# darksim33/Pyneapple

Measured on AMD Instinct MI355X. Metric: voxels/sec (pixelwise triexp LM & 250-bin NNLS) at 1/2/4/8 MI355X, higher is better.
Workload: dtype f64

## Files before the change

pyneapple_amd/csrc/pnx_api.hip:

```cpp
#include <hip/hip_runtime.h>

#include <cmath>
#include <cstdarg>
#include <cstdio>
#include <cstring>
#include <algorithm>
#include <atomic>
#include <chrono>
#include <condition_variable>
#include <cstdlib>
#include <functional>
#include <mutex>
#include <string>
#include <thread>
#include <vector>

#include "pnx_curvefit_f32_kernel.hpp"
#include "pnx_curvefit_kernel.hpp"
#include "pnx_grid.hpp"
#include "pnx_grid_args.hpp"
#include "pnx_grid_posterior.hpp"
#include "pnx_grid_marginal.hpp"
#include "pnx_grid_prior.hpp"
#include "pnx_host_pipeline.hpp"
// ... 30 lines not shown
static constexpr int kQueueRing = 256;
static std::mutex g_mu;
static DeviceInfo g_dev[64];

static int get_device(int device, DeviceInfo **out) {
    int n = 0;
    if (hipGetDeviceCount(&n) != hipSuccess || n <= 0) return set_error(PNX_ERR_NO_DEVICE, "no HIP device visible");
    if (device < 0 || device >= n || device >= 64) return set_error(PNX_ERR_INVALID, "device %d out of range (%d visible)", device, n);
    std::lock_guard<std::mutex> lk(g_mu);
    DeviceInfo &d = g_dev[device];
    if (!d.ok) {
        hipDeviceProp_t prop;
        PNX_HIP(hipGetDeviceProperties(&prop, device));
        d.cus = prop.multiProcessorCount;
        PNX_HIP(hipSetDevice(device));
        PNX_HIP(hipMalloc(&d.queues, sizeof(unsigned long long) * kQueueRing));
        d.ok = true;
    }
    *out = &d;
    return PNX_OK;
}

static int use_device(int device, DeviceInfo **out) {
    if (int rc = get_device(device, out)) return rc;
    PNX_HIP(hipSetDevice(device));
    return PNX_OK;
}

static unsigned long long *next_queue(DeviceInfo *d) {
    std::lock_guard<std::mutex> lk(g_mu);
    unsigned long long *q = d->queues + d->next_queue;
    d->next_queue = (d->next_queue + 1) % kQueueRing;
    return q;
}

struct DevBuf {
    void *p = nullptr;
    ~DevBuf() {
        if (p) (void)hipFree(p);
    }
    int alloc(size_t bytes) {
        hipError_t e = hipMalloc(&p, bytes ? bytes : 8);
        if (e != hipSuccess) return set_error(PNX_ERR_NOMEM, "hipMalloc(%zu): %s", bytes, hipGetErrorString(e));
        return PNX_OK;
    }
};


struct HipBackend {
    typedef hipStream_t stream_t;
    typedef hipEvent_t event_t;
    static bool bind_device(int device) { return hipSetDevice(device) == hipSuccess; }
    static bool stream_create(stream_t *s, bool kernel) {
        int prio_least = 0, prio_greatest = 0;
        if (hipDeviceGetStreamPriorityRange(&prio_least, &prio_greatest) != hipSuccess) return false;
        const int prio_other = prio_least > 0 ? 0 : prio_greatest;
        return hipStreamCreateWithPriority(s, hipStreamNonBlocking, kernel ? prio_least : prio_other) == hipSuccess;
    }
    static void stream_destroy(stream_t s) { (void)hipStreamDestroy(s); }
    static bool stream_sync(stream_t s) { return hipStreamSynchronize(s) == hipSuccess; }
    static bool event_create(event_t *e) { return hipEventCreateWithFlags(e, hipEventDisableTiming) == hipSuccess; }
    static void event_destroy(event_t e) { (void)hipEventDestroy(e); }
    static bool event_record(event_t e, stream_t s) { return hipEventRecord(e, s) == hipSuccess; }
    static bool event_sync(event_t e) { return hipEventSynchronize(e) == hipSuccess; }
};
typedef PipeOpsT<hipStream_t> PipeOps;

static int run_pipeline(int n_chunks, int n_slots, int k_streams, int touchers, int device, hipStream_t user_stream,
                        const PipeOps &ops) {
    return run_pipeline_t<HipBackend>(n_chunks, n_slots, k_streams, touchers, device, user_stream, ops, dev_getenv("PNX_HOST_TRACE") != nullptr);
}

static void touch_pages(void *p, size_t bytes) {
    if (!p || !bytes) return;
    volatile char *c = (volatile char *)p;
    const uintptr_t a = (uintptr_t)p;
    c[0] = 0;
    for (size_t off = (4096 - (a & 4095)) & 4095; off < bytes; off += 4096) c[off] = 0;
}

int env_int(const char *name, int dflt, int lo, int hi) {
    const char *e = getenv(name);
    if (!e) return dflt;
    const long v = atol(e);
    return v < lo ? lo : (v > hi ? hi : (int)v);
}
const char *dev_getenv(const char *name) {
    static const bool enabled = [] {
        const char *e = getenv("PNX_ENABLE_TEST_HOOKS");
        return e && e[0] == '1' && e[1] == 0;
    }();
    return enabled ? getenv(name) : nullptr;
}
int dev_env_int(const char *name, int dflt, int lo, int hi) { return dev_getenv(name) ? env_int(name, dflt, lo, hi) : dflt; }

static std::atomic<int> g_host_calls(0);
struct HostCallGuard {
    int in_flight;
    HostCallGuard() : in_flight(g_host_calls.fetch_add(1) + 1) {}
    ~HostCallGuard() { g_host_calls.fetch_sub(1); }
    int touchers() const { return getenv("PNX_HOST_TOUCHERS") ? env_int("PNX_HOST_TOUCHERS", 2, 0, 8) : (in_flight >= 3 ? 0 : (in_flight == 2 ? 1 : 2)); }
    int out_threads() const { return getenv("PNX_STREAM_OUT_THREADS") ? env_int("PNX_STREAM_OUT_THREADS", 2, 1, 4) : (in_flight >= 4 ? 1 : 2); }
};

struct Carver {
    char *base = nullptr;
    size_t off = 0;
    void *take(size_t bytes) {
        void *p = base ? base + off : nullptr;
        off += (bytes + 255) & ~(size_t)255;
        return p;
    }
};

static int model_n_params(int model) {
    switch (model) {
    case PNX_MODEL_MONO: return 2;
    case PNX_MODEL_BI_REDUCED: return 3;
    case PNX_MODEL_BI_S0: return 4;
    case PNX_MODEL_BI_FULL: return 4;
    case PNX_MODEL_TRI_REDUCED: return 5;
    case PNX_MODEL_TRI_S0: return 6;
    case PNX_MODEL_TRI_FULL: return 6;
    }
    return -1;
}

typedef int (*launch_fn)(int, int, const CurvefitArgs *, int, void *);
static launch_fn g_launch[7] = {pnx_launch_curvefit_m0, pnx_launch_curvefit_m1, pnx_launch_curvefit_m2,
                                pnx_launch_curvefit_m3, pnx_launch_curvefit_m4, pnx_launch_curvefit_m5,
                                pnx_launch_curvefit_m6};

struct StreamLaunch {
    StreamCtl *ctl = nullptr;
    unsigned int *host_flags = nullptr;
    int granule_shift = 0;
    unsigned int spins = 0;
    int phase = 0;
};

static int curvefit_device(const pnx_curvefit_opts *o, int64_t n_vox, const double *b, const double *y_d,
                           const double *p0, const double *lo, const double *hi, const double *fixed, double *popt_d,
                           double *pcov_d, int8_t *status_d, int32_t *nfev_d, double *cost_d, DeviceInfo *dev,
                           hipStream_t stream, const StreamLaunch *sl = nullptr, const int32_t *order = nullptr) {
    CurvefitArgs a;
    memset(&a, 0, sizeof(a));
    if (sl) {
        a.ctl = sl->ctl;
        a.host_flags = sl->host_flags;
        a.granule_shift = sl->granule_shift;
        a.stream_spins = sl->spins;
        a.phase = sl->phase;
    }
    a.order = sl ? nullptr : order;
    a.y = y_d;
    a.popt = popt_d;
    a.pcov = pcov_d;
    a.status = status_d;
    a.nfev = nfev_d;
    a.cost = cost_d;
    a.n_vox = n_vox;
    a.n_b = o->n_b;
    a.per_voxel = o->per_voxel_p0_bounds;
    a.fixed_per_voxel = o->fixed_per_voxel;
    a.max_nfev = o->max_nfev > 0 ? o->max_nfev : 100 * o->n_free;
    a.n_fixed = o->n_fixed;
    a.t1_mode = o->t1_mode;
    a.tr = o->tr;
    a.tm = o->tm;
    a.ftol = o->ftol;
    a.xtol = o->xtol;
    a.gtol = o->gtol;
    for (int k = 0; k < o->n_free; ++k) a.free_idx[k] = o->free_idx[k];
    for (int k = 0; k < o->n_fixed; ++k) a.fixed_idx[k] = o->fixed_idx[k];
    for (int i = 0; i < o->n_b; ++i) a.b[i] = b[i];
    a.absolute_sigma = o->absolute_sigma != 0;
    a.use_sigma = o->sigma != nullptr;
    if (o->sigma)
        for (int i = 0; i < o->n_b; ++i) a.w[i] = 1.0 / o->sigma[i];
    if (o->per_voxel_p0_bounds) {
        a.p0 = p0;
        a.lo = lo;
        a.hi = hi;
    } else {
        for (int k = 0; k < o->n_free; ++k) {
            a.p0s[k] = p0[k];
            a.los[k] = lo[k];
            a.his[k] = hi[k];
        }
    }
    if (o->n_fixed) {
        if (o->fixed_per_voxel)
            a.fixed = fixed;
        else
            for (int k = 0; k < o->n_fixed; ++k) a.fixeds[k] = fixed[k];
    }
    if (a.phase != 2) {
        a.queue = next_queue(dev);
        PNX_HIP(hipMemsetAsync(a.queue, 0, sizeof(unsigned long long), stream));
    }
    return g_launch[o->model](o->n_free, o->jac_mode, &a, dev->cus, (void *)stream);
}

static int check_curvefit_opts(const pnx_curvefit_opts *o) {
    if (!o) return set_error(PNX_ERR_INVALID, "opts is NULL");
    int n_all = model_n_params(o->model);
    if (n_all < 0) return set_error(PNX_ERR_INVALID, "unknown model %d", o->model);
    if (o->t1_mode < 0 || o->t1_mode > 2) return set_error(PNX_ERR_INVALID, "t1_mode %d", o->t1_mode);
    if (o->t1_mode) n_all += 1;
    if (o->n_b < 1 || o->n_b > PNX_MAX_BVALUES) return set_error(PNX_ERR_INVALID, "n_b=%d out of range [1,%d]", o->n_b, PNX_MAX_BVALUES);
    if (o->n_free < 1 || o->n_fixed < 0 || o->n_free + o->n_fixed != n_all)
        return set_error(PNX_ERR_INVALID, "n_free=%d + n_fixed=%d != %d parameters of model %d", o->n_free, o->n_fixed, n_all, o->model);
    bool seen[PNX_MAX_PARAMS] = {false};
    for (int k = 0; k < o->n_free; ++k) {
        const int j = o->free_idx[k];
        if (j < 0 || j >= n_all || seen[j] || (k && j <= o->free_idx[k - 1]))
            return set_error(PNX_ERR_INVALID, "free_idx must be ascending, unique positions in [0,%d)", n_all);
        seen[j] = true;
    }
    for (int k = 0; k < o->n_fixed; ++k) {
        const int j = o->fixed_idx[k];
        if (j < 0 || j >= n_all || seen[j]) return set_error(PNX_ERR_INVALID, "fixed_idx overlaps free_idx or is out of range");
        seen[j] = true;
    }
    if (o->jac_mode != PNX_JAC_FD && o->jac_mode != PNX_JAC_ANALYTIC) return set_error(PNX_ERR_INVALID, "jac_mode %d", o->jac_mode);
    if (o->jac_mode == PNX_JAC_FD && o->n_fixed)
        return set_error(PNX_ERR_UNSUPPORTED,
                         "finite-difference Jacobian with fixed parameters: the reference uses the analytic Jacobian "
                         "there (curvefit.py:274-288); pass PNX_JAC_ANALYTIC");
    if (!(o->ftol >= 0) || !(o->xtol >= 0) || !(o->gtol >= 0)) return set_error(PNX_ERR_INVALID, "tolerances must be >= 0");
    return PNX_OK;
}

}

using namespace pnx;

extern "C" {

int pnx_version(void) { return PNX_VERSION_MAJOR * 100 + PNX_VERSION_MINOR; }

int pnx_device_count(void) {
    int n = 0;
    if (hipGetDeviceCount(&n) != hipSuccess) return 0;
    return n;
}

int pnx_last_error(char *buf, int n) {
    const int len = (int)strlen(g_err);
    if (buf && n > 0) {
        strncpy(buf, g_err, (size_t)n - 1);
        buf[n - 1] = 0;
    }
    return len;
}

int pnx_model_n_params(int model) {
    const int n = model_n_params(model);
    return n < 0 ? set_error(PNX_ERR_INVALID, "unknown model %d", model) : n;
}

}

template <typename S, typename D> __global__ void cvt_kernel(const S *__restrict__ src, D *__restrict__ dst, size_t n) {
    for (size_t i = (size_t)blockIdx.x * blockDim.x + threadIdx.x; i < n; i += (size_t)gridDim.x * blockDim.x)
        dst[i] = (D)src[i];
}
template <typename S, typename D> static int cvt(const S *src, D *dst, size_t n, hipStream_t st) {
    if (!n) return PNX_OK;
    size_t blocks = (n + 255) / 256;
    if (blocks > 16384) blocks = 16384;
    hipLaunchKernelGGL((cvt_kernel<S, D>), dim3((unsigned)blocks), dim3(256), 0, st, src, dst, n);
    PNX_HIP(hipGetLastError());
    return PNX_OK;
}

struct AsyncBuf {
    void *p = nullptr;
    hipStream_t st = nullptr;
    int alloc(size_t bytes, hipStream_t s) {
        st = s;
        hipError_t e = hipMallocAsync(&p, bytes ? bytes : 8, s);
        if (e != hipSuccess) return set_error(PNX_ERR_NOMEM, "hipMallocAsync(%zu): %s", bytes, hipGetErrorString(e));
        return PNX_OK;
    }
    ~AsyncBuf() {
        if (p) (void)hipFreeAsync(p, st);
    }
};

struct DevSet {
    void *dev[ArrayTable::kMax] = {};
    void *xfer[ArrayTable::kMax] = {};
    double *d(int k) const { return (double *)dev[k]; }
};
enum class Carve { Staged, Results, CallerDevice };
static void carve(Carver &cv, const ArrayTable &A, size_t cap, DevSet &D, Carve mode = Carve::Staged, size_t v0 = 0) {
    for (int k = 0; k < A.n; ++k) {
        const HostArray &a = A.a[k];
        D.dev[k] = D.xfer[k] = nullptr;
        if (mode == Carve::CallerDevice) {
            if (!a.host) continue;
            D.xfer[k] = (char *)a.host + v0 * a.w * a.esize;
            D.dev[k] = a.widen ? cv.take(cap * a.w * sizeof(double)) : D.xfer[k];
        } else if ((a.host || a.always) && (a.out || mode == Carve::Staged)) {
            D.dev[k] = cv.take(cap * a.w * (a.widen ? sizeof(double) : a.esize));
// ... 1606 lines not shown
```

pyneapple_amd/csrc/pnx_curvefit_kernel.hpp:

```cpp
#pragma once
#include <hip/hip_runtime.h>
#include <stdint.h>

#include "pnx_trf_math.hpp"

namespace pnx {

constexpr int kWave = 64;
constexpr int kMaxB = 128;
constexpr int kMaxP = 8;
#ifdef PNX_ROW_BLK
template <int N> constexpr int row_blk() { return PNX_ROW_BLK; }
#else
template <int N> constexpr int row_blk() { return N >= 7 ? 2 : (N >= 5 ? 4 : 8); }
#endif
constexpr double kEps = TrfTraits<double>::eps;
constexpr double kSqrtEps = 1.4901161193847656e-08;
template <bool B> struct BoolC {
    static constexpr bool value = B;
};
typedef __attribute__((address_space(3))) void lds_void;

struct StreamCtl {
    unsigned long long ready;
    unsigned int abort;
    unsigned int timed_out;
    unsigned int done[1];
};

struct CurvefitArgs {
    const double *y;
    const double *p0;
    const double *lo;
    const double *hi;
    const double *fixed;
    double *popt;
    double *pcov;
    int8_t *status;
    int32_t *nfev;
    double *cost;
    unsigned long long *queue;
    const int32_t *order;
    StreamCtl *ctl;
    unsigned int *host_flags;
    int granule_shift;
    unsigned int stream_spins;
    int phase;
    long long n_vox;
    int n_b;
    int per_voxel;
    int fixed_per_voxel;
    int max_nfev;
    int n_fixed;
    int t1_mode;
    double tr, tm;
    double ftol, xtol, gtol;
    double p0s[kMaxP], los[kMaxP], his[kMaxP], fixeds[kMaxP];
    int free_idx[kMaxP];
    int fixed_idx[kMaxP];
    int use_sigma;
    int absolute_sigma;
    double b[kMaxB];
    double w[kMaxB];
};

template <int MODEL> struct Model;

template <> struct Model<0> {
    static constexpr int NALL = 2, NC = 1;
    __device__ static constexpr int dpos(int c) { return 1; }
    __device__ static double signal(const double *p, const double *E) { return p[0] * E[0]; }
    __device__ static void jac(const double *p, const double *E, double x, double *r) {
        r[0] = E[0];
        r[1] = -x * p[0] * E[0];
    }
};
template <> struct Model<1> {
    static constexpr int NALL = 3, NC = 2;
    __device__ static constexpr int dpos(int c) { return c == 0 ? 1 : 2; }
    __device__ static double signal(const double *p, const double *E) { return p[0] * E[0] + (1 - p[0]) * E[1]; }
    __device__ static void jac(const double *p, const double *E, double x, double *r) {
        r[0] = E[0] - E[1];
        r[1] = -x * p[0] * E[0];
        r[2] = -x * (1 - p[0]) * E[1];
    }
};
template <> struct Model<2> {
    static constexpr int NALL = 4, NC = 2;
    __device__ static constexpr int dpos(int c) { return c == 0 ? 1 : 2; }
    __device__ static double signal(const double *p, const double *E) {
        return p[3] * (p[0] * E[0] + (1 - p[0]) * E[1]);
    }
    __device__ static void jac(const double *p, const double *E, double x, double *r) {
        r[0] = p[3] * (E[0] - E[1]);
        r[1] = -x * p[3] * p[0] * E[0];
        r[2] = -x * p[3] * (1 - p[0]) * E[1];
        r[3] = p[0] * E[0] + (1 - p[0]) * E[1];
    }
};
template <> struct Model<3> {
    static constexpr int NALL = 4, NC = 2;
    __device__ static constexpr int dpos(int c) { return c == 0 ? 1 : 3; }
    __device__ static double signal(const double *p, const double *E) { return p[0] * E[0] + p[2] * E[1]; }
    __device__ static void jac(const double *p, const double *E, double x, double *r) {
        r[0] = E[0];
        r[1] = -x * p[0] * E[0];
        r[2] = E[1];
        r[3] = -x * p[2] * E[1];
    }
};
template <> struct Model<4> {
    static constexpr int NALL = 5, NC = 3;
    __device__ static constexpr int dpos(int c) { return c == 0 ? 1 : (c == 1 ? 3 : 4); }
    __device__ static double signal(const double *p, const double *E) {
        return p[0] * E[0] + p[2] * E[1] + (1 - p[0] - p[2]) * E[2];
    }
    __device__ static void jac(const double *p, const double *E, double x, double *r) {
        const double f3 = 1 - p[0] - p[2];
        r[0] = E[0] - E[2];
        r[1] = -x * p[0] * E[0];
        r[2] = E[1] - E[2];
        r[3] = -x * p[2] * E[1];
        r[4] = -x * f3 * E[2];
    }
};
template <> struct Model<5> {
    static constexpr int NALL = 6, NC = 3;
    __device__ static constexpr int dpos(int c) { return c == 0 ? 1 : (c == 1 ? 3 : 4); }
    __device__ static double signal(const double *p, const double *E) {
        return p[5] * (p[0] * E[0] + p[2] * E[1] + (1 - p[0] - p[2]) * E[2]);
    }
    __device__ static void jac(const double *p, const double *E, double x, double *r) {
        const double f3 = 1 - p[0] - p[2], S0 = p[5];
        r[0] = S0 * (E[0] - E[2]);
        r[1] = -x * S0 * p[0] * E[0];
        r[2] = S0 * (E[1] - E[2]);
        r[3] = -x * S0 * p[2] * E[1];
        r[4] = -x * S0 * f3 * E[2];
        r[5] = p[0] * E[0] + p[2] * E[1] + f3 * E[2];
    }
};
template <> struct Model<6> {
    static constexpr int NALL = 6, NC = 3;
    __device__ static constexpr int dpos(int c) { return c == 0 ? 1 : (c == 1 ? 3 : 5); }
    __device__ static double signal(const double *p, const double *E) {
        return p[0] * E[0] + p[2] * E[1] + p[4] * E[2];
    }
    __device__ static void jac(const double *p, const double *E, double x, double *r) {
        r[0] = E[0];
        r[1] = -x * p[0] * E[0];
        r[2] = E[1];
        r[3] = -x * p[2] * E[1];
        r[4] = E[2];
        r[5] = -x * p[4] * E[2];
    }
};

template <int MODEL> __host__ __device__ constexpr int colperm(int k) {
    constexpr int P[7][6] = {{0, 1, 2, 3, 4, 5}, {2, 0, 1, 3, 4, 5}, {2, 0, 1, 3, 4, 5}, {3, 1, 2, 0, 4, 5},
                             {4, 3, 0, 2, 1, 5}, {4, 3, 0, 2, 1, 5}, {5, 3, 1, 4, 2, 0}};
    return P[MODEL][k];
}

template <int MODEL> __device__ constexpr int comp_of_param(int j) {
    for (int c = 0; c < Model<MODEL>::NC; ++c)
        if (Model<MODEL>::dpos(c) == j) return c;
    return -1;
}

#ifndef PNX_CF_FAST_EXP
#define PNX_CF_FAST_EXP 1
#endif
#ifndef PNX_CF_HINTS
#define PNX_CF_HINTS 1
#endif
#if PNX_CF_HINTS
#define PNX_LIKELY(x) __builtin_expect(!!(x), 1)
#else
#define PNX_LIKELY(x) (x)
#endif
__device__ inline double exp_fast(double x) {
#if PNX_CF_FAST_EXP
    const double k = __builtin_rint(x * 1.4426950408889634);
    double r = fma(k, -0.6931471805599453, x);
    r = fma(k, -2.3190468138462996e-17, r);
    const double r2 = r * r;
    double qe = 2.7630903490112654e-07;
    qe = fma(qe, r2, 2.480149103909504e-05);
    qe = fma(qe, r2, 0.0013888888945916382);
    qe = fma(qe, r2, 0.041666666666519754);
    qe = fma(qe, r2, 0.5000000000000012);
    double qo = 2.502232256764614e-08;
    qo = fma(qo, r2, 2.755751454582531e-06);
    qo = fma(qo, r2, 0.00019841269589115522);
    qo = fma(qo, r2, 0.008333333333455043);
    qo = fma(qo, r2, 0.16666666666666477);
    const double q = fma(r, qo, qe);
    return ldexp(fma(r, fma(r, q, 1.0), 1.0), __double2int_rz(k));
#else
    return exp(x);
#endif
}

enum LaneState : int { ST_IDLE = 0, ST_INIT = 1, ST_RUN = 2, ST_FINAL = 3 };

template <int N> struct Park {
    static constexpr int NR = N * (N + 1) / 2;
    static constexpr bool kParkV = (N <= 5);
    static constexpr int NV = kParkV ? N * N : 0;
    __host__ __device__ static constexpr int per_wave(int tile_rows) { return kWave * (tile_rows + NR + NV); }
    __host__ __device__ static constexpr int per_wave_f64(int n_b) { return kWave * (((n_b + 1) & ~1) + NR + NV); }
};

#ifndef PNX_CF_WAVES_PER_SIMD
#define PNX_CF_WAVES_PER_SIMD 1
#endif
#ifndef PNX_CF_BLOCK_WAVES
#define PNX_CF_BLOCK_WAVES 4
#endif
template <int MODEL, int N, bool FD, bool PV, bool T1, bool STREAM = false>
__global__ void __launch_bounds__(64 * PNX_CF_BLOCK_WAVES, PNX_CF_WAVES_PER_SIMD) curvefit_kernel(const CurvefitArgs A) {
    using M = Model<MODEL>;
    using PK = Park<N>;
    constexpr int NALL = M::NALL;
    constexpr int NP = NALL + (T1 ? 1 : 0);
    constexpr int NC = M::NC;
    constexpr bool HASFIXED = (N != NP);
    static_assert(!(FD && HASFIXED), "finite-difference mode is only built without fixed parameters");
    auto CP = [](int k) constexpr { return (HASFIXED || k >= NALL) ? k : colperm<MODEL>(k); };

    extern __shared__ double smem[];
    const int n_b = A.n_b;
    double *bsh = smem;
    const int lane = threadIdx.x & (kWave - 1);
    const int wave = threadIdx.x / kWave;
    const bool use_w = A.use_sigma != 0;
    const double *wsh = smem + kMaxB;
    double *ytile = smem + (use_w ? 2 * kMaxB : kMaxB) + (size_t)wave * PK::per_wave_f64(n_b);
    double *ysh = ytile + 2 * lane;
    double *rpark = ytile + (size_t)((n_b + 1) & ~1) * kWave + lane;
    double *vpark = rpark + (size_t)PK::NR * kWave;
    for (int i = threadIdx.x; i < n_b; i += blockDim.x) bsh[i] = A.b[i];
    if (use_w)
        for (int i = threadIdx.x; i < n_b; i += blockDim.x) smem[kMaxB + i] = A.w[i];
    double bmax = 0;
    for (int i = 0; i < n_b; ++i) {
        const double ab = fabs(A.b[i]);
        bmax = (ab < INFINITY) ? fmax(bmax, ab) : INFINITY;
    }
    __syncthreads();
    const bool dma_ok = ((reinterpret_cast<uintptr_t>(A.y) & 7) == 0);

    int state = ST_IDLE;
    long long vox = -1;
    unsigned long long ready_seen = 0;
    int pub = 0;
    auto publish = [&](bool all) {
        const int n_gran = (int)((A.n_vox + (1ll << A.granule_shift) - 1) >> A.granule_shift);
        int upto = pub;
        while (upto < n_gran && (all || !__ballot(state != ST_IDLE && (vox >> A.granule_shift) <= upto))) ++upto;
        if (upto == pub) return;
        __builtin_amdgcn_fence(__ATOMIC_RELEASE, "");
        const unsigned int n_waves = gridDim.x * (blockDim.x / kWave);
        if ((threadIdx.x & (kWave - 1)) == __ffsll((unsigned long long)__ballot(1)) - 1) {
            for (int g = pub; g < upto; ++g) {
                const unsigned int old = __hip_atomic_fetch_add(&A.ctl->done[g], 1u, __ATOMIC_ACQ_REL, __HIP_MEMORY_SCOPE_SYSTEM);
                if (old + 1 == n_waves) __hip_atomic_store(&A.host_flags[g], 1u, __ATOMIC_RELEASE, __HIP_MEMORY_SCOPE_SYSTEM);
            }
        }
        pub = upto;
    };
    double x[N], lb[N], ub[N];
    double pfull[NP];
    double g[N];
    double s[N], uf[N], R2[N][N], d[N], g_h[N];
    double Vreg[PK::kParkV ? 1 : N][PK::kParkV ? 1 : N];
    double smax = 0, smin = 0, theta = 0;
    double cost = 0, Delta = 0, alpha = 0;
    int nfev = 0, term = -99;
    bool first = false;
    double xn[N], step_h_norm = 0, step_norm = 0, predicted = 0;
    if (!PV) {
#pragma unroll
        for (int k = 0; k < N; ++k) {
            lb[k] = A.los[k];
            ub[k] = A.his[k];
        }
    }

#ifdef PNX_CF_STAMP
    unsigned long long seg[8] = {0, 0, 0, 0, 0, 0, 0, 0}, act[8] = {0, 0, 0, 0, 0, 0, 0, 0}, cnt[8] = {0, 0, 0, 0, 0, 0, 0, 0};
    unsigned long long tl = __builtin_amdgcn_s_memtime();
#define CFSTAMP(k) do { __builtin_amdgcn_s_waitcnt(0); const unsigned long long t_ = __builtin_amdgcn_s_memtime(); seg[k] += t_ - tl; tl = t_; } while (0)
#define CFACT(k, cond) do { act[k] += __popcll(__ballot(cond)); cnt[k] += 1; } while (0)
#else
#define CFSTAMP(k) do {} while (0)
#define CFACT(k, cond) do {} while (0)
#endif
    auto refill = [&]() {
    while (state == ST_IDLE) {
        const unsigned long long idx = atomicAdd(A.queue, 1ULL);
        if (idx >= (unsigned long long)A.n_vox) break;
        if constexpr (STREAM) {
            if (idx >= ready_seen) {
                bool got = false;
                const unsigned int *abort_word = A.host_flags + ((A.n_vox + (1ll << A.granule_shift) - 1) >> A.granule_shift);
                for (unsigned int spins = 0; spins < A.stream_spins; ++spins) {
                    ready_seen = __hip_atomic_load(&A.ctl->ready, __ATOMIC_ACQUIRE, __HIP_MEMORY_SCOPE_SYSTEM);
                    if (idx < ready_seen) {
                        got = true;
                        break;
                    }
                    if ((spins & 15u) == 15u && __hip_atomic_load(abort_word, __ATOMIC_RELAXED, __HIP_MEMORY_SCOPE_SYSTEM)) break;
                    __builtin_amdgcn_s_sleep(127);
                }
                if (!got) {
                    if (!__hip_atomic_load(abort_word, __ATOMIC_RELAXED, __HIP_MEMORY_SCOPE_SYSTEM))
                        __hip_atomic_store(&A.ctl->timed_out, 1u, __ATOMIC_RELAXED, __HIP_MEMORY_SCOPE_SYSTEM);
                    break;
                }
            }
        }
        vox = (long long)idx;
        if constexpr (!STREAM) {
            if (A.order) vox = A.order[idx];
        }
        const double *yv = A.y + (size_t)vox * n_b;
        if (dma_ok) {
            const int pairs = n_b >> 1;
            for (int c = 0; c < pairs; ++c)
                __builtin_amdgcn_global_load_lds((const void *)(yv + 2 * c), (lds_void *)(ytile + c * 2 * kWave), 16, 0, 0);
            if (n_b & 1) {
                if (vox + 1 < A.n_vox)
                    __builtin_amdgcn_global_load_lds((const void *)(yv + n_b - 1), (lds_void *)(ytile + pairs * 2 * kWave), 16, 0, 0);
                else
                    ysh[pairs * 2 * kWave] = yv[n_b - 1];
            }
        } else {
            for (int i = 0; i < n_b; ++i) ysh[(i >> 1) * 2 * kWave + (i & 1)] = yv[i];
        }
        bool okb = true, okp = true;
        double p0v[N];
#pragma unroll
        for (int k = 0; k < N; ++k) {
            if (PV) {
                p0v[k] = A.p0[(size_t)k * A.n_vox + vox];
                lb[k] = A.lo[(size_t)k * A.n_vox + vox];
                ub[k] = A.hi[(size_t)k * A.n_vox + vox];
            } else
                p0v[k] = A.p0s[k];
            okb = okb && (lb[k] < ub[k]);
            okp = okp && (p0v[k] >= lb[k]) && (p0v[k] <= ub[k]);
        }
        if (HASFIXED) {
#pragma unroll
            for (int j = 0; j < NP; ++j) pfull[j] = 0;
            for (int f = 0; f < A.n_fixed; ++f) {
                const double fv = A.fixed_per_voxel ? A.fixed[(size_t)f * A.n_vox + vox] : A.fixeds[f];
#pragma unroll
                for (int j = 0; j < NP; ++j)
                    if (A.fixed_idx[f] == j) pfull[j] = fv;
            }
        }
        if (!okb || !okp) {
            const int st = !okb ? -1 : -3;
#pragma unroll
            for (int k = 0; k < N; ++k) A.popt[(size_t)k * A.n_vox + vox] = p0v[k];
            if (A.status) A.status[vox] = (int8_t)st;
            if (A.nfev) A.nfev[vox] = 0;
            if (A.cost) A.cost[vox] = NAN;
            continue;
        }
#pragma unroll
        for (int k = 0; k < N; ++k) xn[k] = strictly_feasible_r(p0v[k], lb[k], ub[k]);
        state = ST_INIT;
        nfev = 0;
        term = -99;
        alpha = 0.0;
    }
    };
    refill();
    if constexpr (STREAM) {
        if (!__ballot(state != ST_IDLE)) publish(true);
    }
    for (;;) {
        CFSTAMP(7);
        if (state == ST_IDLE) break;
        asm volatile("s_waitcnt vmcnt(0)" ::: "memory");
        CFSTAMP(0);
        CFACT(1, true);

        double Rn[N][N], qn[N], gn[N], cost_new = 0;
        bool finite_f = true, yfinite = true;
        {
            double pe[NP];
            if (HASFIXED) {
#pragma unroll
                for (int j = 0; j < NP; ++j) {
                    pe[j] = pfull[j];
#pragma unroll
                    for (int k = 0; k < N; ++k)
                        if (A.free_idx[k] == j) pe[j] = xn[k];
                }
            } else {
#pragma unroll
                for (int j = 0; j < NP; ++j) pe[j] = xn[j];
            }
            double dxv[N];
            if (FD) {
#pragma unroll
                for (int k = 0; k < N; ++k) {
                    const double sign = (xn[k] >= 0) ? 1.0 : -1.0;
                    double h = kSqrtEps * sign * fmax(1.0, fabs(xn[k]));
                    const double lower_dist = xn[k] - lb[k], upper_dist = ub[k] - xn[k];
                    const double xx = xn[k] + h;
                    const bool violated = (xx < lb[k]) || (xx > ub[k]);
                    const bool fitting = fabs(h) <= fmax(lower_dist, upper_dist);
                    if (violated && fitting) h = -h;
                    if (!fitting) h = (upper_dist >= lower_dist) ? upper_dist : -lower_dist;
                    dxv[k] = (xn[k] + h) - xn[k];
                }
            }
            double A1 = 1.0, eTM = 1.0, fac = 1.0, dfac = 0.0;
            if (T1) {
                const bool steam = A.t1_mode == 2;
                const double T1v = pe[NALL];
                const double eTR = exp(-A.tr / T1v);
                A1 = 1 - eTR;
                eTM = steam ? exp(-A.tm / T1v) : 1.0;
                fac = A1 * eTM;
                dfac = steam ? eTM / (T1v * T1v) * (-A.tr * eTR + A.tm * A1) : (-eTR * A.tr / (T1v * T1v));
                if (FD) {
                    const double dx = dxv[N - 1];
                    const double T2 = T1v + dx;
                    const double fac2 = (1 - exp(-A.tr / T2)) * (steam ? exp(-A.tm / T2) : 1.0);
                    dfac = (fac2 - fac) / dx;
                }
            }
#pragma unroll
            for (int i = 0; i < N; ++i) {
                qn[i] = 0;
                gn[i] = 0;
#pragma unroll
                for (int j = 0; j < N; ++j) Rn[i][j] = 0;
            }
            constexpr int kRowBlk = row_blk<N>();
            static_assert(kRowBlk % 2 == 0, "a block reads its signal values as [pair][lane][2] pairs");
            auto row_block = [&](auto fastgz_c, auto usew_c, auto tail_c, const int i0) __attribute__((always_inline)) {
                constexpr bool FASTGZ = decltype(fastgz_c)::value, USEW = decltype(usew_c)::value, TAIL = decltype(tail_c)::value;
                double blk[kRowBlk][N + 1];
                double bv[TAIL ? 1 : kRowBlk], yv[TAIL ? 1 : kRowBlk];
                if constexpr (!TAIL) {
#pragma unroll
                    for (int r = 0; r < kRowBlk; r += 2) {
                        const double2 b2 = *reinterpret_cast<const double2 *>(bsh + i0 + r);
                        const double2 y2 = *reinterpret_cast<const double2 *>(ysh + (size_t)(i0 + r) * kWave);
                        bv[r] = b2.x;
                        bv[r + 1] = b2.y;
                        yv[r] = y2.x;
                        yv[r + 1] = y2.y;
                    }
                }
#pragma unroll
                for (int r = 0; r < kRowBlk; ++r) {
                    const bool live = !TAIL || (i0 + r < n_b);
                    const int ii = live ? i0 + r : 0;
                    const double bb = TAIL ? bsh[ii] : bv[TAIL ? 0 : r];
                    const double nb = -bb;
                    const double yi = TAIL ? ysh[(ii >> 1) * 2 * kWave + (ii & 1)] : yv[TAIL ? 0 : r];
                    yfinite = yfinite && isfinite(yi);
                    double E[NC];
#pragma unroll
                    for (int c = 0; c < NC; ++c) E[c] = exp_fast(nb * pe[M::dpos(c)]);
                    const double base = M::signal(pe, E);
                    double r0 = (T1 ? base * A1 * eTM : base) - yi;
                    double jr[N];
                    {
                        double ja[NP];
                        M::jac(pe, E, bb, ja);
                        if (FD) {
#pragma unroll
                            for (int k = 0; k < NALL; ++k) {
                                if (comp_of_param<MODEL>(k) >= 0) {
                                    const double z = nb * dxv[k];
                                    double gz;
#if PNX_CF_FAST_EXP
                                    if (FASTGZ || PNX_LIKELY(fabs(z) < 2e-4))
                                        gz = fma(z, fma(z, fma(z, 1.0 / 24, 1.0 / 6), 0.5), 1.0);
                                    else
#endif
                                    if (fabs(z) < 1e-3)
                                        gz = 1.0 + z * (0.5 + z * (1.0 / 6 + z * (1.0 / 24 + z * (1.0 / 120 + z * (1.0 / 720)))));
                                    else
                                        gz = expm1(z) / z;
                                    ja[k] *= gz;
                                }
                            }
                        }
                        if (T1) {
#pragma unroll
                            for (int k = 0; k < NALL; ++k) ja[k] *= fac;
                            ja[NP - 1] = base * dfac;
                        }
                        if (TAIL ? use_w : USEW) {
                            const double t = wsh[ii];
                            r0 *= t;
#pragma unroll
                            for (int k = 0; k < NP; ++k) ja[k] *= t;
                        }
                        if (HASFIXED) {
#pragma unroll
                            for (int k = 0; k < N; ++k) {
                                jr[k] = 0;
#pragma unroll
                                for (int j = 0; j < NP; ++j)
                                    if (A.free_idx[k] == j) jr[k] = ja[j];
                            }
                        } else {
#pragma unroll
                            for (int k = 0; k < N; ++k) jr[k] = ja[k];
                        }
                    }
                    const double rr = live ? r0 : 0.0;
                    finite_f = finite_f && isfinite(rr);
                    cost_new += rr * rr;
#pragma unroll
                    for (int k = 0; k < N; ++k) {
                        const double jk = live ? jr[k] : 0.0;
                        gn[k] += jk * rr;
                    }
#pragma unroll
                    for (int k = 0; k < N; ++k) blk[r][k] = live ? jr[CP(k)] : 0.0;
                    blk[r][N] = rr;
                }
                CFSTAMP(1);
                qr_merge<N, kRowBlk>(Rn, qn, blk);
                CFSTAMP(6);
            };
            auto row_loop = [&](auto fastgz_c, auto usew_c) __attribute__((always_inline)) {
                int i0 = 0;
                for (; i0 + kRowBlk <= n_b; i0 += kRowBlk) row_block(fastgz_c, usew_c, BoolC<false>{}, i0);
                if (i0 < n_b) row_block(BoolC<false>{}, BoolC<false>{}, BoolC<true>{}, i0);
            };
            constexpr bool kOneLoop = (N >= 6);
            bool gz_cubic = FD && PNX_CF_FAST_EXP && !kOneLoop;
            if (FD && PNX_CF_FAST_EXP && !kOneLoop) {
                bool in_range = true;
#pragma unroll
                for (int k = 0; k < NALL; ++k)
                    if (comp_of_param<MODEL>(k) >= 0) in_range = in_range && (fabs(bmax * dxv[k]) < 2e-4);
                gz_cubic = __ballot(!in_range) == 0;
            }
            if constexpr (kOneLoop) {
                for (int i0 = 0; i0 < n_b; i0 += kRowBlk) row_block(BoolC<false>{}, BoolC<false>{}, BoolC<true>{}, i0);
            } else if (PNX_LIKELY(!use_w && (gz_cubic || !FD))) {
                if constexpr (FD && PNX_CF_FAST_EXP)
                    row_loop(BoolC<true>{}, BoolC<false>{});
                else
                    row_loop(BoolC<false>{}, BoolC<false>{});
            } else if (use_w) {
                row_loop(BoolC<false>{}, BoolC<true>{});
            } else {
                if constexpr (FD) row_loop(BoolC<false>{}, BoolC<false>{});
            }
            cost_new *= 0.5;
        }

        CFSTAMP(1);
        bool accepted = false;
        int final_status = 0;
        if (state == ST_INIT) {
            if (!finite_f) {
                final_status = yfinite ? -4 : -2;
                cost = NAN;
                nfev = 0;
                state = ST_FINAL;
            } else {
                accepted = true;
                nfev = 1;
                first = true;
                state = ST_RUN;
            }
        } else {
            nfev += 1;
            if (!finite_f) {
                Delta = 0.25 * step_h_norm;
            } else {
                const double actual = cost - cost_new;
                double ratio;
                if (predicted > 0)
                    ratio = actual / predicted;
                else if (predicted == 0 && actual == 0)
                    ratio = 1;
                else
                    ratio = 0;
                double Delta_new = Delta;
                if (ratio < 0.25)
                    Delta_new = 0.25 * step_h_norm;
                else if (ratio > 0.75 && step_h_norm > 0.95 * Delta)
                    Delta_new = Delta * 2.0;
                const bool ftol_ok = (actual < A.ftol * cost) && (ratio > 0.25);
                const bool xtol_ok = step_norm < A.xtol * (A.xtol + normn<N>(x));
                if (ftol_ok && xtol_ok)
                    term = 4;
                else if (ftol_ok)
                    term = 2;
                else if (xtol_ok)
                    term = 3;
                if (term == -99) {
                    alpha *= Delta / Delta_new;
                    Delta = Delta_new;
                }
                accepted = actual > 0;
            }
        }
        if (accepted) {
#pragma unroll
            for (int i = 0; i < N; ++i) {
                x[i] = xn[i];
                g[i] = gn[i];
            }
            cost = cost_new;
            int t = 0;
#pragma unroll
            for (int i = 0; i < N; ++i)
#pragma unroll
                for (int j = i; j < N; ++j) rpark[(t++) * kWave] = Rn[i][j];
        }

        double v[N], dv[N], g_norm = 0;
        if (state == ST_RUN && (accepted || term != -99 || nfev >= A.max_nfev)) {
#pragma unroll
            for (int i = 0; i < N; ++i) {
                v[i] = 1.0;
                dv[i] = 0.0;
                if (g[i] < 0 && isfinite(ub[i])) {
                    v[i] = ub[i] - x[i];
                    dv[i] = -1;
                }
                if (g[i] > 0 && isfinite(lb[i])) {
                    v[i] = x[i] - lb[i];
                    dv[i] = 1;
                }
                g_norm = fmax(g_norm, fabs(g[i] * v[i]));
            }
            if (first) {
                double t = 0;
#pragma unroll
                for (int i = 0; i < N; ++i) {
                    const double q = x[i] / sqrt(v[i]);
                    t += q * q;
                }
                Delta = sqrt(t);
                if (Delta == 0) Delta = 1.0;
                first = false;
            }
            if (g_norm < A.gtol) term = 1;
            if (term != -99 || nfev >= A.max_nfev) {
                final_status = (term == -99) ? 0 : term;
                state = ST_FINAL;
            }
        }

        CFSTAMP(2);
        CFACT(3, state == ST_FINAL);
        if (state == ST_FINAL) {
            const bool ok = final_status > 0;
#pragma unroll
            for (int k = 0; k < N; ++k) {
                const double pk = ok ? x[k] : (PV ? A.p0[(size_t)k * A.n_vox + vox] : A.p0s[k]);
                A.popt[(size_t)k * A.n_vox + vox] = pk;
            }
            if (A.status) A.status[vox] = (int8_t)final_status;
            if (A.nfev) A.nfev[vox] = nfev;
            if (A.cost) A.cost[vox] = cost;
            if (A.pcov && ok) {
                double *pc = A.pcov + (size_t)vox * N * N;
#pragma unroll
                for (int t = 0; t < PK::NR; ++t) pc[t] = rpark[t * kWave];
            }
            state = ST_IDLE;
        }
        CFACT(0, state == ST_IDLE);
        if constexpr (STREAM) {
            const bool any_idle = __ballot(state == ST_IDLE) != 0;
            if (state == ST_IDLE) refill();
            if (any_idle) publish(false);
        } else {
            if (state == ST_IDLE) refill();
        }

        CFSTAMP(3);
        CFACT(4, state == ST_RUN && accepted);
        CFACT(5, state == ST_RUN);
        if (state == ST_RUN) {
            if (accepted) {
                double diag_h[N];
#pragma unroll
                for (int i = 0; i < N; ++i) {
                    d[i] = sqrt(v[i]);
                    diag_h[i] = g[i] * dv[i];
                    g_h[i] = d[i] * g[i];
                }
                double q2[N];
                double blk[N][N + 1];
#pragma unroll
                for (int i = 0; i < N; ++i) {
                    q2[i] = qn[i];
#pragma unroll
                    for (int j = 0; j < N; ++j) {
                        R2[i][j] = (j >= i) ? Rn[i][j] * d[CP(j)] : 0.0;
                        blk[i][j] = (i == j) ? sqrt(diag_h[CP(i)]) : 0.0;
                    }
                    blk[i][N] = 0.0;
                }
                qr_merge<N, N>(R2, q2, blk);
                double W[N][N], Vw[N][N];
#pragma unroll
                for (int i = 0; i < N; ++i)
#pragma unroll
                    for (int j = 0; j < N; ++j) W[i][j] = (i >= j) ? R2[j][i] : 0.0;
                jacobi_svd<N>(W, Vw);
                smax = 0;
                smin = INFINITY;
#pragma unroll
                for (int k = 0; k < N; ++k) {
                    double nn = 0, dq = 0;
#pragma unroll
                    for (int i = 0; i < N; ++i) {
                        nn += W[i][k] * W[i][k];
                        dq += Vw[i][k] * q2[i];
                    }
                    double inv = 0.0;
                    if (nn > 0) nn = fast_sqrt_rsqrt(nn, &inv);
                    s[k] = nn;
                    uf[k] = dq;
#pragma unroll
                    for (int i = 0; i < N; ++i) {
                        if (PK::kParkV)
                            vpark[(i * N + k) * kWave] = W[i][k] * inv;
                        else
                            Vreg[PK::kParkV ? 0 : i][PK::kParkV ? 0 : k] = W[i][k] * inv;
                    }
                    smax = fmax(smax, nn);
                    smin = fmin(smin, nn);
                }
                theta = fmax(0.995, 1 - g_norm);
            }
            CFSTAMP(4);
            double V[N][N];
#pragma unroll
            for (int i = 0; i < N; ++i)
#pragma unroll
                for (int k = 0; k < N; ++k)
                    V[i][k] = PK::kParkV ? vpark[(i * N + k) * kWave] : Vreg[PK::kParkV ? 0 : i][PK::kParkV ? 0 : k];
            double xP[N], lbP[N], ubP[N], dP[N], ghP[N];
#pragma unroll
            for (int i = 0; i < N; ++i) {
                xP[i] = x[CP(i)];
                lbP[i] = lb[CP(i)];
                ubP[i] = ub[CP(i)];
                dP[i] = d[CP(i)];
                ghP[i] = g_h[CP(i)];
            }
            double p_h[N], p[N], step[N], step_h[N];
            alpha = solve_lsq_trust_region<N>(n_b, uf, s, V, smax, smin, Delta, alpha, p_h);
#pragma unroll
            for (int i = 0; i < N; ++i) p[i] = dP[i] * p_h[i];
            predicted = select_step<N>(xP, R2, ghP, p, p_h, dP, Delta, lbP, ubP, theta, step, step_h);
#pragma unroll
            for (int i = 0; i < N; ++i) xn[CP(i)] = strictly_feasible0(xP[i] + step[i], lbP[i], ubP[i]);
            step_h_norm = normn<N>(step_h);
            step_norm = normn<N>(step);
            CFSTAMP(5);
        }
    }
#ifdef PNX_CF_STAMP
    if (threadIdx.x == 0 && blockIdx.x == 3)
        printf("CFSTAMP refill=%llu pass_rows=%llu pass_qr_merge=%llu D+Blight=%llu final=%llu Bheavy=%llu C=%llu loop=%llu | iters=%llu idle_at_top=%.2f final=%.2f Bheavy=%.2f run=%.2f\n",
               seg[0], seg[1], seg[6], seg[2], seg[3], seg[4], seg[5], seg[7], cnt[1], (double)act[0] / cnt[0], (double)act[3] / cnt[3],
               (double)act[4] / cnt[4], (double)act[5] / cnt[5]);
#endif
}

struct ColPerm {
    int p[kMaxP];
};

template <int N>
__global__ void __launch_bounds__(256) pcov_kernel(double *pcov, const int8_t *status, const double *cost,
                                                   long long n_vox, int n_b, const ColPerm cp, int absolute_sigma) {
    const long long vox = (long long)blockIdx.x * blockDim.x + threadIdx.x;
    if (vox >= n_vox) return;
    double *pc = pcov + (size_t)vox * N * N;
    if (status[vox] <= 0) {
#pragma unroll
        for (int k = 0; k < N * N; ++k) pc[k] = NAN;
        return;
    }
    double W[N][N], Vw[N][N];
    {
        int t = 0;
#pragma unroll
        for (int i = 0; i < N; ++i)
#pragma unroll
            for (int j = 0; j < N; ++j) W[i][j] = 0.0;
#pragma unroll
        for (int i = 0; i < N; ++i)
#pragma unroll
            for (int j = i; j < N; ++j) W[j][i] = pc[t++];
    }
    jacobi_svd<N>(W, Vw);
    double s2[N], sm = 0;
#pragma unroll
    for (int k = 0; k < N; ++k) {
        double nn = 0;
#pragma unroll
        for (int i = 0; i < N; ++i) nn += W[i][k] * W[i][k];
        s2[k] = nn;
        sm = fmax(sm, nn);
    }
    const double thr = kEps * (n_b > N ? n_b : N) * sqrt(sm);
    const bool dof = absolute_sigma || n_b > N;
    const double s_sq = absolute_sigma ? 1.0 : (dof ? 2.0 * cost[vox] / (double)(n_b - N) : 0.0);
    double wgt[N];
#pragma unroll
    for (int k = 0; k < N; ++k) wgt[k] = (sqrt(s2[k]) > thr) ? 1.0 / (s2[k] * s2[k]) : 0.0;
    bool bad = false;
    double out[N][N];
#pragma unroll
    for (int i = 0; i < N; ++i)
#pragma unroll
        for (int j = 0; j < N; ++j) {
            double a = 0;
#pragma unroll
            for (int k = 0; k < N; ++k) a += W[i][k] * W[j][k] * wgt[k];
            out[i][j] = a;
            bad = bad || isnan(a);
        }
#pragma unroll
    for (int i = 0; i < N; ++i)
#pragma unroll
        for (int j = 0; j < N; ++j) pc[cp.p[i] * N + cp.p[j]] = (bad || !dof) ? INFINITY : out[i][j] * s_sq;
}

}
```

Baseline: 127.6 million.

## Add wave-team tail mode where idle lanes compute rows for the last voxel

When only one lane in a wavefront still has a live voxel and the queue is empty, the kernel switches to a team mode. All 64 lanes broadcast the owner's parameters, each evaluates a subset of the b-value rows (residual and Jacobian) into LDS, and the owner then consumes the rows through the usual QR merge. This targets the tail where a wave runs at 1/64 utilisation on straggler voxels. The cost is LDS round-trips, readlane broadcasts and a larger kernel body. The mode is gated by a PNX_CF_TEAM environment variable (default on) and applies only to non-stream kernels with N<=5.

```diff
diff --git a/pyneapple_amd/csrc/pnx_api.hip b/pyneapple_amd/csrc/pnx_api.hip
--- a/pyneapple_amd/csrc/pnx_api.hip
+++ b/pyneapple_amd/csrc/pnx_api.hip
@@ -206,6 +206,7 @@
         a.stream_spins = sl->spins;
         a.phase = sl->phase;
     }
+    a.team = dev_env_int("PNX_CF_TEAM", 1, 0, 1);
     a.order = sl ? nullptr : order;
     a.y = y_d;
     a.popt = popt_d;
diff --git a/pyneapple_amd/csrc/pnx_curvefit_kernel.hpp b/pyneapple_amd/csrc/pnx_curvefit_kernel.hpp
--- a/pyneapple_amd/csrc/pnx_curvefit_kernel.hpp
+++ b/pyneapple_amd/csrc/pnx_curvefit_kernel.hpp
@@ -46,6 +46,7 @@
     int granule_shift;
     unsigned int stream_spins;
     int phase;
+    int team;
     long long n_vox;
     int n_b;
     int per_voxel;
@@ -202,6 +203,12 @@
 #endif
 }
 
+__device__ inline double lane_bcast(double v, int src) {
+    const unsigned long long u = __builtin_bit_cast(unsigned long long, v);
+    const unsigned int lo = __builtin_amdgcn_readlane((int)(unsigned int)u, src), hi = __builtin_amdgcn_readlane((int)(unsigned int)(u >> 32), src);
+    return __builtin_bit_cast(double, ((unsigned long long)hi << 32) | lo);
+}
+
 enum LaneState : int { ST_IDLE = 0, ST_INIT = 1, ST_RUN = 2, ST_FINAL = 3 };
 
 template <int N> struct Park {
@@ -289,9 +296,10 @@
     }
 
 #ifdef PNX_CF_STAMP
-    unsigned long long seg[8] = {0, 0, 0, 0, 0, 0, 0, 0}, act[8] = {0, 0, 0, 0, 0, 0, 0, 0}, cnt[8] = {0, 0, 0, 0, 0, 0, 0, 0};
+    unsigned long long seg[9] = {0, 0, 0, 0, 0, 0, 0, 0, 0}, act[9] = {0, 0, 0, 0, 0, 0, 0, 0, 0}, cnt[9] = {0, 0, 0, 0, 0, 0, 0, 0, 0};
     unsigned long long tl = __builtin_amdgcn_s_memtime();
-#define CFSTAMP(k) do { __builtin_amdgcn_s_waitcnt(0); const unsigned long long t_ = __builtin_amdgcn_s_memtime(); seg[k] += t_ - tl; tl = t_; } while (0)
+    bool cf_in_team = false;
+#define CFSTAMP(k) do { __builtin_amdgcn_s_waitcnt(0); const unsigned long long t_ = __builtin_amdgcn_s_memtime(); if ((k) == 8 || !cf_in_team) { seg[k] += t_ - tl; tl = t_; } } while (0)
 #define CFACT(k, cond) do { act[k] += __popcll(__ballot(cond)); cnt[k] += 1; } while (0)
 #else
 #define CFSTAMP(k) do {} while (0)
@@ -383,9 +391,8 @@
     if constexpr (STREAM) {
         if (!__ballot(state != ST_IDLE)) publish(true);
     }
-    for (;;) {
-        CFSTAMP(7);
-        if (state == ST_IDLE) break;
+    auto iterate = [&](auto team_c, const int owner) __attribute__((always_inline)) {
+        constexpr bool TM = decltype(team_c)::value;
         asm volatile("s_waitcnt vmcnt(0)" ::: "memory");
         CFSTAMP(0);
         CFACT(1, true);
@@ -393,6 +400,20 @@
         double Rn[N][N], qn[N], gn[N], cost_new = 0;
         bool finite_f = true, yfinite = true;
         {
+            if constexpr (TM) {
+#pragma unroll
+                for (int k = 0; k < N; ++k) {
+                    xn[k] = lane_bcast(xn[k], owner);
+                    if (PV) {
+                        lb[k] = lane_bcast(lb[k], owner);
+                        ub[k] = lane_bcast(ub[k], owner);
+                    }
+                }
+                if (HASFIXED) {
+#pragma unroll
+                    for (int j = 0; j < NP; ++j) pfull[j] = lane_bcast(pfull[j], owner);
+                }
+            }
             double pe[NP];
             if (HASFIXED) {
 #pragma unroll
@@ -424,7 +445,7 @@
             double A1 = 1.0, eTM = 1.0, fac = 1.0, dfac = 0.0;
             if (T1) {
                 const bool steam = A.t1_mode == 2;
-                const double T1v = pe[NALL];
+                const double T1v = pe[T1 ? NALL : 0];
                 const double eTR = exp(-A.tr / T1v);
                 A1 = 1 - eTR;
                 eTM = steam ? exp(-A.tm / T1v) : 1.0;
@@ -446,8 +467,78 @@
             }
             constexpr int kRowBlk = row_blk<N>();
             static_assert(kRowBlk % 2 == 0, "a block reads its signal values as [pair][lane][2] pairs");
+            auto row_eval = [&](auto fastgz_c, auto usew_c, auto tail_c, const int ii, const double bb, const double yi, double &r0_out,
+                                double (&jr)[N]) __attribute__((always_inline)) {
+                constexpr bool FASTGZ = decltype(fastgz_c)::value, USEW = decltype(usew_c)::value, TAIL = decltype(tail_c)::value;
+                const double nb = -bb;
+                double E[NC];
+#pragma unroll
+                for (int c = 0; c < NC; ++c) E[c] = exp_fast(nb * pe[M::dpos(c)]);
+                const double base = M::signal(pe, E);
+                double r0 = (T1 ? base * A1 * eTM : base) - yi;
+                {
+                    double ja[NP];
+                    M::jac(pe, E, bb, ja);
+                    if (FD) {
+#pragma unroll
+                        for (int k = 0; k < NALL; ++k) {
+                            if (comp_of_param<MODEL>(k) >= 0) {
+                                const double z = nb * dxv[k];
+                                double gz;
+#if PNX_CF_FAST_EXP
+                                if (FASTGZ || PNX_LIKELY(fabs(z) < 2e-4))
+                                    gz = fma(z, fma(z, fma(z, 1.0 / 24, 1.0 / 6), 0.5), 1.0);
+                                else
+#endif
+                                if (fabs(z) < 1e-3)
+                                    gz = 1.0 + z * (0.5 + z * (1.0 / 6 + z * (1.0 / 24 + z * (1.0 / 120 + z * (1.0 / 720)))));
+                                else
+                                    gz = expm1(z) / z;
+                                ja[k] *= gz;
+                            }
+                        }
+                    }
+                    if (T1) {
+#pragma unroll
+                        for (int k = 0; k < NALL; ++k) ja[k] *= fac;
+                        ja[NP - 1] = base * dfac;
+                    }
+                    if (TAIL ? use_w : USEW) {
+                        const double t = wsh[ii];
+                        r0 *= t;
+#pragma unroll
+                        for (int k = 0; k < NP; ++k) ja[k] *= t;
+                    }
+                    if (HASFIXED) {
+#pragma unroll
+                        for (int k = 0; k < N; ++k) {
+                            jr[k] = 0;
+#pragma unroll
+                            for (int j = 0; j < NP; ++j)
+                                jr[k] = (A.free_idx[k] == j) ? ja[j] : jr[k];
+                        }
+                    } else {
+#pragma unroll
+                        for (int k = 0; k < N; ++k) jr[k] = ja[k];
+                    }
+                }
+                r0_out = r0;
+            };
+            auto row_consume = [&](double (&brow)[N + 1], const bool live, const double r0, const double (&jr)[N]) __attribute__((always_inline)) {
+                const double rr = live ? r0 : 0.0;
+                finite_f = finite_f && isfinite(rr);
+                cost_new += rr * rr;
+#pragma unroll
+                for (int k = 0; k < N; ++k) {
+                    const double jk = live ? jr[k] : 0.0;
+                    gn[k] += jk * rr;
+                }
+#pragma unroll
+                for (int k = 0; k < N; ++k) brow[k] = live ? jr[CP(k)] : 0.0;
+                brow[N] = rr;
+            };
             auto row_block = [&](auto fastgz_c, auto usew_c, auto tail_c, const int i0) __attribute__((always_inline)) {
-                constexpr bool FASTGZ = decltype(fastgz_c)::value, USEW = decltype(usew_c)::value, TAIL = decltype(tail_c)::value;
+                constexpr bool TAIL = decltype(tail_c)::value;
                 double blk[kRowBlk][N + 1];
                 double bv[TAIL ? 1 : kRowBlk], yv[TAIL ? 1 : kRowBlk];
                 if constexpr (!TAIL) {
@@ -466,72 +557,11 @@
                     const bool live = !TAIL || (i0 + r < n_b);
                     const int ii = live ? i0 + r : 0;
                     const double bb = TAIL ? bsh[ii] : bv[TAIL ? 0 : r];
-                    const double nb = -bb;
                     const double yi = TAIL ? ysh[(ii >> 1) * 2 * kWave + (ii & 1)] : yv[TAIL ? 0 : r];
                     yfinite = yfinite && isfinite(yi);
-                    double E[NC];
-#pragma unroll
-                    for (int c = 0; c < NC; ++c) E[c] = exp_fast(nb * pe[M::dpos(c)]);
-                    const double base = M::signal(pe, E);
-                    double r0 = (T1 ? base * A1 * eTM : base) - yi;
-                    double jr[N];
-                    {
-                        double ja[NP];
-                        M::jac(pe, E, bb, ja);
-                        if (FD) {
-#pragma unroll
-                            for (int k = 0; k < NALL; ++k) {
-                                if (comp_of_param<MODEL>(k) >= 0) {
-                                    const double z = nb * dxv[k];
-                                    double gz;
-#if PNX_CF_FAST_EXP
-                                    if (FASTGZ || PNX_LIKELY(fabs(z) < 2e-4))
-                                        gz = fma(z, fma(z, fma(z, 1.0 / 24, 1.0 / 6), 0.5), 1.0);
-                                    else
-#endif
-                                    if (fabs(z) < 1e-3)
-                                        gz = 1.0 + z * (0.5 + z * (1.0 / 6 + z * (1.0 / 24 + z * (1.0 / 120 + z * (1.0 / 720)))));
-                                    else
-                                        gz = expm1(z) / z;
-                                    ja[k] *= gz;
-                                }
-                            }
-                        }
-                        if (T1) {
-#pragma unroll
-                            for (int k = 0; k < NALL; ++k) ja[k] *= fac;
-                            ja[NP - 1] = base * dfac;
-                        }
-                        if (TAIL ? use_w : USEW) {
-                            const double t = wsh[ii];
-                            r0 *= t;
-#pragma unroll
-                            for (int k = 0; k < NP; ++k) ja[k] *= t;
-                        }
-                        if (HASFIXED) {
-#pragma unroll
-                            for (int k = 0; k < N; ++k) {
-                                jr[k] = 0;
-#pragma unroll
-                                for (int j = 0; j < NP; ++j)
-                                    if (A.free_idx[k] == j) jr[k] = ja[j];
-                            }
-                        } else {
-#pragma unroll
-                            for (int k = 0; k < N; ++k) jr[k] = ja[k];
-                        }
-                    }
-                    const double rr = live ? r0 : 0.0;
-                    finite_f = finite_f && isfinite(rr);
-                    cost_new += rr * rr;
-#pragma unroll
-                    for (int k = 0; k < N; ++k) {
-                        const double jk = live ? jr[k] : 0.0;
-                        gn[k] += jk * rr;
-                    }
-#pragma unroll
-                    for (int k = 0; k < N; ++k) blk[r][k] = live ? jr[CP(k)] : 0.0;
-                    blk[r][N] = rr;
+                    double r0, jr[N];
+                    row_eval(fastgz_c, usew_c, tail_c, ii, bb, yi, r0, jr);
+                    row_consume(blk[r], live, r0, jr);
                 }
                 CFSTAMP(1);
                 qr_merge<N, kRowBlk>(Rn, qn, blk);
@@ -551,7 +581,48 @@
                     if (comp_of_param<MODEL>(k) >= 0) in_range = in_range && (fabs(bmax * dxv[k]) < 2e-4);
                 gz_cubic = __ballot(!in_range) == 0;
             }
-            if constexpr (kOneLoop) {
+            if constexpr (TM) {
+                static_assert(N + 1 <= 8 && 2 * kWave == kMaxB, "a team row is 8 doubles; two rows per lane cover every n_b");
+                double *trow = ytile + (owner < kWave / 2 ? kWave : 0);
+                const double *yown = ytile + 2 * owner;
+                bool ybad = false;
+                __builtin_amdgcn_fence(__ATOMIC_ACQ_REL, "wavefront");
+#pragma unroll
+                for (int h = 0; h < kMaxB / kWave; ++h) {
+                    if (h * kWave < n_b) {
+                        const int i = lane + h * kWave;
+                        const bool live = i < n_b;
+                        const int ii = live ? i : 0;
+                        const double yi = yown[(ii >> 1) * 2 * kWave + (ii & 1)];
+                        ybad = ybad || !isfinite(yi);
+                        double r0, jr[N];
+                        row_eval(BoolC<false>{}, BoolC<false>{}, BoolC<true>{}, ii, bsh[ii], yi, r0, jr);
+                        if (live) {
+                            double *tr = trow + (i >> 1) * 2 * kWave + (i & 1) * 8;
+#pragma unroll
+                            for (int k = 0; k < N; ++k) tr[k] = jr[k];
+                            tr[N] = r0;
+                        }
+                    }
+                }
+                yfinite = __ballot(ybad) == 0;
+                __builtin_amdgcn_fence(__ATOMIC_ACQ_REL, "wavefront");
+                __builtin_amdgcn_wave_barrier();
+                for (int i0 = 0; i0 < n_b; i0 += kRowBlk) {
+                    double blk[kRowBlk][N + 1];
+#pragma unroll
+                    for (int r = 0; r < kRowBlk; ++r) {
+                        const bool live = i0 + r < n_b;
+                        const int ii = live ? i0 + r : 0;
+                        const double *tr = trow + (ii >> 1) * 2 * kWave + (ii & 1) * 8;
+                        double jr[N];
+#pragma unroll
+                        for (int k = 0; k < N; ++k) jr[k] = tr[k];
+                        row_consume(blk[r], live, tr[N], jr);
+                    }
+                    qr_merge<N, kRowBlk>(Rn, qn, blk);
+                }
+            } else if constexpr (kOneLoop) {
                 for (int i0 = 0; i0 < n_b; i0 += kRowBlk) row_block(BoolC<false>{}, BoolC<false>{}, BoolC<true>{}, i0);
             } else if (PNX_LIKELY(!use_w && (gz_cubic || !FD))) {
                 if constexpr (FD && PNX_CF_FAST_EXP)
@@ -567,6 +638,9 @@
         }
 
         CFSTAMP(1);
+        if constexpr (TM) {
+            if (state == ST_IDLE) return;
+        }
         bool accepted = false;
         int final_status = 0;
         if (state == ST_INIT) {
@@ -686,7 +760,7 @@
             const bool any_idle = __ballot(state == ST_IDLE) != 0;
             if (state == ST_IDLE) refill();
             if (any_idle) publish(false);
-        } else {
+        } else if constexpr (!TM) {
             if (state == ST_IDLE) refill();
         }
 
@@ -774,11 +848,33 @@
             step_norm = normn<N>(step);
             CFSTAMP(5);
         }
+    };
+    constexpr bool kTeam = !STREAM && N <= 5;
+    constexpr int kTeamMax = 1;
+    for (;;) {
+        CFSTAMP(7);
+        if (state == ST_IDLE) break;
+        if constexpr (kTeam) {
+            if (!PNX_LIKELY(__popcll(__ballot(1)) > kTeamMax || !A.team)) break;
+        }
+        iterate(BoolC<false>{}, 0);
+    }
+    if constexpr (kTeam) {
+#ifdef PNX_CF_STAMP
+        cf_in_team = true;
+#endif
+        for (;;) {
+            const unsigned long long livem = __ballot(state != ST_IDLE);
+            if (!livem) break;
+            iterate(BoolC<true>{}, __ffsll(livem) - 1);
+            CFSTAMP(8);
+            CFACT(8, true);
+        }
     }
 #ifdef PNX_CF_STAMP
     if (threadIdx.x == 0 && blockIdx.x == 3)
-        printf("CFSTAMP refill=%llu pass_rows=%llu pass_qr_merge=%llu D+Blight=%llu final=%llu Bheavy=%llu C=%llu loop=%llu | iters=%llu idle_at_top=%.2f final=%.2f Bheavy=%.2f run=%.2f\n",
-               seg[0], seg[1], seg[6], seg[2], seg[3], seg[4], seg[5], seg[7], cnt[1], (double)act[0] / cnt[0], (double)act[3] / cnt[3],
+        printf("CFSTAMP refill=%llu pass_rows=%llu pass_qr_merge=%llu D+Blight=%llu final=%llu Bheavy=%llu C=%llu loop=%llu team=%llu | iters=%llu team_iters=%llu idle_at_top=%.2f final=%.2f Bheavy=%.2f run=%.2f\n",
+               seg[0], seg[1], seg[6], seg[2], seg[3], seg[4], seg[5], seg[7], seg[8], cnt[1], cnt[8], (double)act[0] / cnt[0], (double)act[3] / cnt[3],
                (double)act[4] / cnt[4], (double)act[5] / cnt[5]);
 #endif
 }
```

After: 136.7 million, median of 6. +7.1%, better.
